# bensonlzl/spaced-kmer-sketching

Measured on AMD Instinct MI355X. Metric: k-mers hashed/s + genome-pairs ANI/s at 1/2/4/8 MI355X; % HBM roofline, higher is better.
Workload: dtype u64; 1 GPU; config3: 1x3 Gb multi-contig genome per GPU, spaced seed w=31/k=21 (mask seed 0), FracMinHash 1/1000; builds_in_flight=3, genome_bytes=3000000024, windows_per_genome=2999036400, sketch_size=2998764, parallelism=genome-sharded x1

## Files before the change

spaced-kmer-sketching_amd/csrc/scan.hip:

```cpp
#include <hip/hip_runtime.h>

#include <cstdlib>

#include <cstdint>
#include <type_traits>

#include "code_objects.hpp"
#include "scan.hpp"
#include "sks_hash.hpp"

namespace sks {

namespace {

constexpr int kBlock = 256;
constexpr int kWPT = 16;
constexpr int kTile = kBlock * kWPT;
constexpr int kHaloWords = 4;
constexpr int kWords = kBlock + kHaloWords;
constexpr int kLoadVecs = (kWords * 16 + 16) / 16;
constexpr int kQCap = 2048;
#ifndef SKS_SCAN_QCAP
#define SKS_SCAN_QCAP 512
#endif
template <int MODE>
constexpr int qcap() { return MODE == kModeList ? kQCap : SKS_SCAN_QCAP; }
constexpr unsigned char kSep = '\n';

struct Geom {
  uint64_t win0;
  uint64_t seg_end;
  uint32_t seg;
};

__device__ __forceinline__ Geom tile_geom(const ScanParams& p, uint64_t tile, uint32_t& seg) {
  while (seg + 1 < p.n_seg && tile >= p.tile_prefix[seg + 1]) ++seg;
  Geom g;
  g.seg = seg;
  g.win0 = p.seg_begin[seg] + (tile - p.tile_prefix[seg]) * (uint64_t)kTile;
  g.seg_end = p.seg_end[seg];
  return g;
}

__device__ __forceinline__ uint4 load_vec(const uint8_t* __restrict__ seq, int64_t base, int k,
                                          int64_t seg_end) {
  int64_t a = base + 16 * (int64_t)k;
  if (a + 16 <= seg_end) return *reinterpret_cast<const uint4*>(seq + a);
  uint32_t wv[4];
#pragma unroll
  for (int q = 0; q < 4; ++q) {
    uint32_t v = 0;
#pragma unroll
    for (int b = 0; b < 4; ++b) {
      int64_t pos = a + 4 * q + b;
      uint32_t ch = pos < seg_end ? seq[pos] : kSep;
      v |= ch << (8 * b);
    }
    wv[q] = v;
  }
  return make_uint4(wv[0], wv[1], wv[2], wv[3]);
}

__device__ __forceinline__ uint32_t align_shift(const uint8_t* seq, uint64_t win0) {
  return (uint32_t)(((uintptr_t)seq + win0) & 15u);
}

__device__ __forceinline__ void encode4(uint32_t x, uint32_t& le8, uint32_t& inv4) {
  uint32_t low = x | 0x20202020u;
  uint32_t code = ((low >> 1) ^ (low >> 2)) & 0x03030303u;
  uint32_t expect = __builtin_amdgcn_perm(0u, 0x74676361u, code);
  uint32_t eq = expect ^ low;
  uint32_t t = (eq & 0x7F7F7F7Fu) + 0x7F7F7F7Fu;
  t = ~(t | eq | 0x7F7F7F7Fu);
  uint32_t bad = (~t) & 0x80808080u;
  inv4 = (bad * 0x00204081u) >> 28;
  uint32_t y = code | (code >> 6);
  le8 = (y | (y >> 12)) & 0xFFu;
}

__device__ __forceinline__ uint32_t funnel(uint32_t hi, uint32_t lo, uint32_t s) {
  return __builtin_amdgcn_alignbit(hi, lo, s);
}

template <bool ALIGNED>
__device__ __forceinline__ void pack16(const uint32_t (&x)[5], uint32_t sb, uint32_t& le,
                                       uint32_t& inv) {
  uint32_t w[4], g[4], sad = 0;
#pragma unroll
  for (int k = 0; k < 4; ++k) {
    w[k] = ALIGNED ? x[k] : funnel(x[k + 1], x[k], sb);
    const uint32_t low = w[k] | 0x20202020u;
    const uint32_t code = ((low >> 1) ^ (low >> 2)) & 0x03030303u;
    const uint32_t expect = __builtin_amdgcn_perm(0u, 0x74676361u, code);
    sad = __builtin_amdgcn_sad_u8(low, expect, sad);
    g[k] = code * 0x01041040u;
  }
  const uint32_t g01 = __builtin_amdgcn_perm(g[1], g[0], 0x0c0c0703u);
  const uint32_t g23 = __builtin_amdgcn_perm(g[3], g[2], 0x0c0c0703u);
  le = __builtin_amdgcn_perm(g23, g01, 0x05040100u);
  inv = 0;
  if (sad) {
#pragma unroll
    for (int k = 0; k < 4; ++k) {
      uint32_t le8, inv4;
      encode4(w[k], le8, inv4);
      inv |= inv4 << (4 * k);
    }
  }
}

__device__ __forceinline__ uint32_t rev_pairs(uint32_t x) {
  uint32_t r = __builtin_bitreverse32(x);
  return ((r >> 1) & 0x55555555u) | ((r & 0x55555555u) << 1);
}


__device__ __forceinline__ unsigned long long wave_aggregated_inc(unsigned long long* counter) {
  const uint64_t act = __ballot(true);
  const uint32_t rank = __builtin_amdgcn_mbcnt_hi((uint32_t)(act >> 32),
                                                  __builtin_amdgcn_mbcnt_lo((uint32_t)act, 0u));
  unsigned long long base = 0;
  if (rank == 0) base = atomicAdd(counter, (unsigned long long)__popcll(act));
  const uint32_t lo = __builtin_amdgcn_readfirstlane((uint32_t)base);
  const uint32_t hi = __builtin_amdgcn_readfirstlane((uint32_t)(base >> 32));
  return (((unsigned long long)hi << 32) | lo) + rank;
}

template <int MODE>
struct Queue {
  uint64_t key[qcap<MODE>()];
  uint64_t val[MODE == kModeBottom ? qcap<MODE>() : 1];
  uint32_t n;
  unsigned long long base;
  unsigned long long wins;
};

template <int MODE>
__device__ __forceinline__ void emit(const ScanParams& p, Queue<MODE>& q, uint32_t seg,
                                     uint64_t key, uint64_t val) {
  uint32_t slot = atomicAdd(&q.n, 1u);
  if (slot < (uint32_t)qcap<MODE>()) {
    q.key[slot] = key;
    if constexpr (MODE == kModeBottom) q.val[slot] = val;
  } else {
    unsigned long long g = wave_aggregated_inc(&p.seg_count[seg]);
    if (g < p.seg_out_cap[seg]) {
      uint64_t o = p.seg_out_off[seg] + g;
      p.out_key[o] = key;
      if constexpr (MODE == kModeBottom) p.out_val[o] = val;
    }
  }
}

template <int MODE>
__device__ __forceinline__ void flush(const ScanParams& p, Queue<MODE>& q, uint32_t seg) {
  __syncthreads();
  if (threadIdx.x == 0 && q.wins) atomicAdd(&p.seg_windows[seg], q.wins);
  constexpr uint32_t cap = qcap<MODE>();
  uint32_t n = q.n < cap ? q.n : cap;
  if (n) {
    if (threadIdx.x == 0) q.base = atomicAdd(&p.seg_count[seg], (unsigned long long)n);
    __syncthreads();
    uint64_t base = q.base;
    uint64_t cap = p.seg_out_cap[seg];
    uint64_t off = p.seg_out_off[seg];
    for (uint32_t i = threadIdx.x; i < n; i += kBlock) {
      if (base + i < cap) {
        p.out_key[off + base + i] = q.key[i];
        if constexpr (MODE == kModeBottom) p.out_val[off + base + i] = q.val[i];
      }
    }
  }
  __syncthreads();
  if (threadIdx.x == 0) {
    q.n = 0;
    q.wins = 0;
  }
  __syncthreads();
}

__device__ __forceinline__ void add_windows(unsigned long long& wins, uint32_t cnt) {
  uint32_t v = cnt;
#pragma unroll
  for (int o = 32; o > 0; o >>= 1) v += __shfl_xor(v, o, 64);
  if ((threadIdx.x & 63) == 0 && v) atomicAdd(&wins, (unsigned long long)v);
}

template <int FLAVOUR>
__device__ __forceinline__ uint64_t fmh_narrow(const ScanParams& p, uint64_t c) {
  uint64_t h;
  if constexpr (FLAVOUR == 0) {
    h = hash_mix(c + kGolden32);
    h = hash_mix(h + kGolden32);
    h = hash_mix(h + (128 + kGolden32));
  } else {
    h = hash_bitset128<1>(c, 0);
  }
  return h ^ p.kconst;
}

__device__ __forceinline__ uint64_t mix3_head(uint64_t c) {
  uint64_t h = hash_mix(c + kGolden32);
  h = hash_mix(h + kGolden32);
  uint64_t x = h + (128 + kGolden32);
  x ^= x >> 32;
  x = mul_const<kMixMul>(x);
  return x ^ (x >> 32);
}

template <int MODE>
__device__ __forceinline__ bool keep_fmh(const ScanParams& p, uint64_t f, uint64_t thresh) {
  if constexpr (MODE != kModeBottom) return div_test(f, p.low_mask, p.high_mask, p.dinv, p.dlim);
  else return f <= thresh;
}

constexpr int kBeOff = 2;

template <int MODE, int PRE>
constexpr int min_waves() {
#ifdef SKS_SCAN_MIN_WAVES
  return SKS_SCAN_MIN_WAVES;
#else
  return PRE ? 7 : MODE == kModeList ? 4 : 5;
#endif
}

constexpr uint32_t kCandCap = 128;

constexpr int kFminMaxW = 31;
__device__ __forceinline__ uint64_t min_below_2_62(uint64_t a, uint64_t b) {
  uint64_t r;
  asm("v_min_f64 %0, %1, %2" : "=v"(r) : "v"(a), "v"(b));
  return r;
}

template <int MODE, int FLAVOUR, int PRE = 0, int FMIN = 0>
__global__ __launch_bounds__(kBlock, (min_waves<MODE, PRE>())) void scan_kernel(ScanParams p) {
  __shared__ uint32_t s_raw[kLoadVecs * 4];
  __shared__ uint32_t s_be[kWords + 2 + kBeOff];
  __shared__ uint32_t s_lc[kWords + 2];
  __shared__ uint32_t s_inv[kWords + 2];
  __shared__ Queue<MODE> q;
  __shared__ ulonglong2 s_cand[PRE ? (kBlock / 64) * kCandCap : 1];
  __shared__ uint32_t s_ctop[PRE ? kBlock / 64 : 1];

  __shared__ unsigned long long s_next;

  const int tid = threadIdx.x;
  const bool dyn = p.tile_queue != nullptr;
  uint64_t t_begin, t_end;
  if (dyn) {
    t_begin = (uint64_t)blockIdx.x * p.chunk;
    t_end = min(t_begin + p.chunk, p.n_tiles);
  } else {
    t_begin = (uint64_t)blockIdx.x * p.n_tiles / gridDim.x;
    t_end = (uint64_t)(blockIdx.x + 1) * p.n_tiles / gridDim.x;
  }
  if (tid == 0) {
    q.n = 0;
    q.wins = 0;
  }
  if (t_begin >= t_end) return;
  unsigned long long grab = 0;

  const int w = p.w;
  const uint32_t dshift = 2 * (32 - w);
  const uint64_t wmask_bits = (w >= 64) ? ~0ull : ((1ull << w) - 1);
  if (tid < kBeOff) s_be[tid] = 0;
  const uint32_t r = tid & 15;
  const uint32_t wbase = (uint32_t)(tid >> 4) * kWPT;
  const uint32_t of = 2 * r + 64 - dshift;
  const uint32_t qf = (of - 1) >> 5;
  const uint32_t sF = 32 * qf + 32 - of;
  const uint32_t sR = 2 * r;
  const uint32_t* const fb = s_be + (kBeOff - 2) + wbase + qf;
  const uint32_t* const rb = s_lc + wbase;

  uint32_t seg_lo = 0, seg_hi = p.n_seg;
  while (seg_lo + 1 < seg_hi) {
    uint32_t mid = (seg_lo + seg_hi) >> 1;
    if (p.tile_prefix[mid] <= t_begin) seg_lo = mid; else seg_hi = mid;
  }
  uint32_t cur_seg = seg_lo, pf_seg = seg_lo;

  Geom pg = tile_geom(p, t_begin, pf_seg);
  int64_t pf_base = (int64_t)pg.win0 - align_shift(p.seq, pg.win0);
  uint4 v0 = load_vec(p.seq, pf_base, tid, (int64_t)pg.seg_end);
  uint4 v1 = make_uint4(0, 0, 0, 0);
  if (tid < kLoadVecs - kBlock) v1 = load_vec(p.seq, pf_base, kBlock + tid, (int64_t)pg.seg_end);

  uint32_t win_count = 0;
  uint32_t count_seg = cur_seg;

  for (uint64_t tile = t_begin; tile < t_end;) {
    Geom g = tile_geom(p, tile, cur_seg);
    if (g.seg != count_seg) {
      add_windows(q.wins, win_count);
      win_count = 0;
      flush<MODE>(p, q, count_seg);
      count_seg = g.seg;
    }
    const uint32_t shift = align_shift(p.seq, g.win0);
    const uint64_t thresh = (MODE == kModeBottom) ? p.seg_thresh[g.seg] : 0;
    const bool last_of_chunk = tile + 1 == t_end;
    if (dyn && tid == 0) {
      if (tile == t_begin)
        grab = (unsigned long long)gridDim.x * p.chunk + atomicAdd(p.tile_queue, (unsigned long long)p.chunk);
      if (last_of_chunk) s_next = grab;
    }

    auto store_word = [&](int i, uint32_t le, uint32_t inv) {
      s_be[kBeOff + i] = rev_pairs(le);
      s_lc[i] = ~le;
      s_inv[i] = inv;
    };
    if (shift == 0) {
      uint32_t le, inv;
      const uint32_t x0[5] = {v0.x, v0.y, v0.z, v0.w, 0u};
      pack16<true>(x0, 0, le, inv);
      store_word(tid, le, inv);
      if (tid < kHaloWords) {
        const uint32_t x1[5] = {v1.x, v1.y, v1.z, v1.w, 0u};
        pack16<true>(x1, 0, le, inv);
        store_word(kBlock + tid, le, inv);
      }
    } else {
      reinterpret_cast<uint4*>(s_raw)[tid] = v0;
      if (tid < kLoadVecs - kBlock) reinterpret_cast<uint4*>(s_raw)[kBlock + tid] = v1;
      __syncthreads();
      const uint32_t sb = (shift & 3) * 8;
      for (int i = tid; i < kWords; i += kBlock) {
        const uint32_t wi = (16 * i + shift) >> 2;
        uint32_t x[5];
#pragma unroll
        for (int k = 0; k < 5; ++k) x[k] = s_raw[wi + k];
        uint32_t le, inv;
        pack16<false>(x, sb, le, inv);
        store_word(i, le, inv);
      }
    }
    __syncthreads();
    uint64_t next_tile = !last_of_chunk ? tile + 1 : p.n_tiles;
    if (last_of_chunk && dyn) {
      const unsigned long long sn = s_next;
      next_tile = ((uint64_t)__builtin_amdgcn_readfirstlane((uint32_t)(sn >> 32)) << 32) |
                  __builtin_amdgcn_readfirstlane((uint32_t)sn);
    }

    if (next_tile < (dyn ? p.n_tiles : t_end)) {
      Geom ng = tile_geom(p, next_tile, pf_seg);
      pf_base = (int64_t)ng.win0 - align_shift(p.seq, ng.win0);
      v0 = load_vec(p.seq, pf_base, tid, (int64_t)ng.seg_end);
      if (tid < kLoadVecs - kBlock) v1 = load_vec(p.seq, pf_base, kBlock + tid, (int64_t)ng.seg_end);
    }

    const int lane = tid & 63;
    bool dirty = s_inv[tid] != 0;
    if (lane < 2) dirty = dirty || s_inv[(tid | 63) + 1 + lane] != 0;
    const bool wave_clean = !__any(dirty);
    auto canon_of = [&](uint32_t fh, uint32_t fl, uint32_t rh, uint32_t rl) -> uint64_t {
      const uint64_t F = (((uint64_t)fh) << 32) | fl;
      const uint64_t R = (((uint64_t)rh) << 32) | rl;
      const uint64_t fm = F & p.mask_lo, rm = R & p.mask_lo;
      if constexpr (FMIN) return min_below_2_62(fm, rm);
      else return fm < rm ? fm : rm;
    };
    auto canon_at = [&](uint32_t m) -> uint64_t {
      const uint32_t f0 = fb[m], f1 = fb[m + 1], f2 = fb[m + 2];
      const uint32_t r0 = rb[m], r1 = rb[m + 1], r2 = rb[m + 2];
      return canon_of(funnel(f0, f1, sF), funnel(f1, f2, sF), funnel(r2, r1, sR), funnel(r1, r0, sR));
    };
    auto for_windows_checked = [&](auto body) {
      const uint32_t* const ib = s_inv + wbase;
      uint32_t fw = fb[1], rw = rb[1];
      uint32_t fp = funnel(fb[0], fw, sF), rp = funnel(rw, rb[0], sR);
      uint32_t i0 = ib[0], i1 = ib[1];
      uint32_t fnext = 0, rnext = 0, inext = 0;
      if constexpr (!PRE) {
        fnext = fb[2];
        rnext = rb[2];
        inext = ib[2];
      }
#pragma unroll 1
      for (int m = 0; m < kWPT; ++m) {
        uint32_t fw2, rw2, i2;
        if constexpr (PRE) {
          fw2 = fb[m + 2];
          rw2 = rb[m + 2];
          i2 = ib[m + 2];
        } else {
          fw2 = fnext;
          rw2 = rnext;
          i2 = inext;
          fnext = fb[m + 3];
          rnext = rb[m + 3];
          inext = ib[m + 3];
        }
        const uint32_t fn = funnel(fw, fw2, sF), rn = funnel(rw2, rw, sR);
        const uint64_t iv = (uint64_t)i0 | ((uint64_t)i1 << 16) | ((uint64_t)i2 << 32);
        body(m, canon_of(fp, fn, rn, rp), ((iv >> r) & wmask_bits) == 0);
        fw = fw2; rw = rw2; fp = fn; rp = rn; i0 = i1; i1 = i2;
      }
    };
    auto for_windows = [&](auto body) {
      uint32_t fw = fb[1], rw = rb[1];
      uint32_t fp = funnel(fb[0], fw, sF), rp = funnel(rw, rb[0], sR);
      uint32_t fnext = fb[2], rnext = rb[2];
#pragma unroll
      for (int m = 0; m < kWPT; ++m) {
        const uint32_t fw2 = fnext, rw2 = rnext;
        if (m + 1 < kWPT) {
          fnext = fb[m + 3];
          rnext = rb[m + 3];
        }
        asm volatile("" ::: "memory");
        const uint32_t fn = funnel(fw, fw2, sF), rn = funnel(rw2, rw, sR);
        body(m, canon_of(fp, fn, rn, rp));
        fw = fw2; rw = rw2; fp = fn; rp = rn;
      }
    };
    if constexpr (PRE) {
      const uint32_t wv = __builtin_amdgcn_readfirstlane(tid >> 6);
      ulonglong2* cb = s_cand + wv * kCandCap;
      uint32_t* const ctop = s_ctop + wv;
      typedef unsigned long long u64x2 __attribute__((ext_vector_type(2)));
      typedef __attribute__((address_space(3))) u64x2 lds_u64x2;
      const uint32_t cb_lds = (uint32_t)(uintptr_t)(__attribute__((address_space(3))) void*)cb;
      auto set_cursor = [&](uint32_t n) {
        if (lane == 0) *ctop = cb_lds + 16 * n;
        __builtin_amdgcn_fence(__ATOMIC_RELEASE, "wavefront");
        __builtin_amdgcn_wave_barrier();
        __builtin_amdgcn_fence(__ATOMIC_ACQUIRE, "wavefront");
      };
      const uint32_t pmask = p.low_mask & 0xFu;
      const uint32_t kbits = (uint32_t)p.kconst & pmask;
      const uint32_t rest_lo = p.low_mask & ~0xFu, rest_hi = p.high_mask;
      uint32_t cnt = 0;
      set_cursor(0);
      auto finish = [&](uint32_t n) {
        __builtin_amdgcn_wave_barrier();
        if ((uint32_t)lane < n) {
          const ulonglong2 e = cb[lane];
          uint64_t y = mul_const<kMixMul>(e.x);
          y ^= y >> 28;
          const uint64_t f = y ^ p.kconst;
          bool keep = mul_uniform(f, p.dinv) <= p.dlim;
          if (rest_lo | rest_hi)
            keep = keep && ((((uint32_t)f & rest_lo) | ((uint32_t)(f >> 32) & rest_hi)) == 0);
          if (keep) emit<MODE>(p, q, g.seg, e.y, 0);
        }
        __builtin_amdgcn_wave_barrier();
      };
      auto window_pre = [&](uint64_t c, bool valid) {
          const uint64_t z = mix3_head(c);
          const uint32_t ylo = (uint32_t)z * (uint32_t)kMixMul;
          const bool pass = (((ylo ^ (ylo >> 28)) & pmask) == kbits) && valid;
          const uint64_t bal = __ballot(pass);
          if (pass) {
            const uint32_t slot = atomicAdd(ctop, 16u);
            u64x2 zc;
            zc.x = z;
            zc.y = c;
            *(lds_u64x2*)(uintptr_t)slot = zc;
          }
          cnt += (uint32_t)__popcll(bal);
          if (cnt >= 64) {
            finish(64);
            const uint32_t rest = cnt - 64;
            ulonglong2 t = make_ulonglong2(0, 0);
            if ((uint32_t)lane < rest) t = cb[64 + lane];
            __builtin_amdgcn_wave_barrier();
            if ((uint32_t)lane < rest) cb[lane] = t;
            cnt = rest;
            set_cursor(rest);
          }
      };
      if (wave_clean) {
        for_windows([&](int, uint64_t c) { window_pre(c, true); });
        win_count += kWPT;
      } else {
        for_windows_checked([&](int, uint64_t c, bool valid) {
          win_count += valid ? 1u : 0u;
          window_pre(c, valid);
        });
      }
      if (cnt) finish(cnt);
    } else {
    uint32_t keepmask = 0;
    const uint32_t thr_top = (uint32_t)(thresh >> 36);
    const uint32_t k_top = (uint32_t)(p.kconst >> 32);
    auto keep_window = [&](uint64_t c) -> bool {
      if constexpr (MODE == kModeBottom && FLAVOUR == 0) {
        const uint64_t y = mul_const<kMixMul>(mix3_head(c));
        return (((uint32_t)(y >> 32) ^ k_top) >> 4) <= thr_top;
      } else {
        return keep_fmh<MODE>(p, fmh_narrow<FLAVOUR>(p, c), thresh);
      }
    };
    if (wave_clean) {
      for_windows([&](int m, uint64_t c) { keepmask |= (keep_window(c) ? 1u : 0u) << m; });
      win_count += kWPT;
    } else {
      for_windows_checked([&](int m, uint64_t c, bool valid) {
        win_count += valid ? 1u : 0u;
        keepmask |= (keep_window(c) && valid ? 1u : 0u) << m;
      });
    }
    while (keepmask) {
      const uint32_t j = __builtin_ctz(keepmask);
      keepmask &= keepmask - 1;
      if constexpr (MODE == kModeList) {
        emit<MODE>(p, q, g.seg, g.win0 + (uint64_t)(16 * (wbase + j) + r), 0);
      } else {
        const uint64_t c = canon_at(j);
        if constexpr (MODE == kModeFrac) emit<MODE>(p, q, g.seg, c, 0);
        else emit<MODE>(p, q, g.seg, c, c);
      }
    }
    }

    __syncthreads();
    if (q.n >= (uint32_t)qcap<MODE>() / 2) {
      add_windows(q.wins, win_count);
      win_count = 0;
      flush<MODE>(p, q, g.seg);
    }
    if (!last_of_chunk) {
      ++tile;
    } else if (dyn) {
      t_begin = tile = next_tile;
      t_end = min(next_tile + p.chunk, p.n_tiles);
    } else {
      break;
    }
  }
  add_windows(q.wins, win_count);
  flush<MODE>(p, q, count_seg);
}

template <int MODE, int FLAVOUR>
__global__ __launch_bounds__(kBlock) void scan_kernel_wide(ScanParams p) {
  __shared__ uint32_t s_raw[kLoadVecs * 4];
  __shared__ uint32_t s_be[kWords + 2];
  __shared__ uint32_t s_lc[kWords + 2];
  __shared__ uint32_t s_inv[kWords + 2];
  __shared__ uint64_t q_a[kQCap / 2], q_b[kQCap / 2], q_c[kQCap / 2];
  __shared__ uint32_t q_n;
  __shared__ unsigned long long q_base, q_wins;

  const int tid = threadIdx.x;
  const uint64_t t_begin = (uint64_t)blockIdx.x * p.n_tiles / gridDim.x;
  const uint64_t t_end = (uint64_t)(blockIdx.x + 1) * p.n_tiles / gridDim.x;
  if (tid == 0) {
    q_n = 0;
    q_wins = 0;
  }
  if (t_begin >= t_end) return;
  constexpr uint32_t cap = kQCap / 2;

  const int w = p.w;
  const uint32_t fshift = 128 - 2 * w;
  const uint64_t wmask_bits = (w >= 64) ? ~0ull : ((1ull << w) - 1);

  uint32_t seg_lo = 0, seg_hi = p.n_seg;
  while (seg_lo + 1 < seg_hi) {
    uint32_t mid = (seg_lo + seg_hi) >> 1;
    if (p.tile_prefix[mid] <= t_begin) seg_lo = mid; else seg_hi = mid;
  }
  uint32_t cur_seg = seg_lo, pf_seg = seg_lo;
  Geom pg = tile_geom(p, t_begin, pf_seg);
  int64_t pf_base = (int64_t)pg.win0 - align_shift(p.seq, pg.win0);
  uint4 v0 = load_vec(p.seq, pf_base, tid, (int64_t)pg.seg_end);
  uint4 v1 = make_uint4(0, 0, 0, 0);
  if (tid < kLoadVecs - kBlock) v1 = load_vec(p.seq, pf_base, kBlock + tid, (int64_t)pg.seg_end);
  uint32_t win_count = 0;
  uint32_t count_seg = cur_seg;

  auto wflush = [&](uint32_t seg) {
    __syncthreads();
    if (tid == 0 && q_wins) atomicAdd(&p.seg_windows[seg], q_wins);
    uint32_t n = q_n < cap ? q_n : cap;
    if (n) {
      if (tid == 0) q_base = atomicAdd(&p.seg_count[seg], (unsigned long long)n);
      __syncthreads();
      uint64_t base = q_base, c = p.seg_out_cap[seg], off = p.seg_out_off[seg];
      for (uint32_t i = tid; i < n; i += kBlock)
        if (base + i < c) {
          p.out_key[off + base + i] = q_a[i];
          if (MODE != kModeList) p.out_val[off + base + i] = q_b[i];
          if (MODE == kModeBottom) p.out_hi[off + base + i] = q_c[i];
        }
    }
    __syncthreads();
    if (tid == 0) {
      q_n = 0;
      q_wins = 0;
    }
    __syncthreads();
  };

  for (uint64_t tile = t_begin; tile < t_end; ++tile) {
    Geom g = tile_geom(p, tile, cur_seg);
    if (g.seg != count_seg) {
      add_windows(q_wins, win_count);
      win_count = 0;
      wflush(count_seg);
      count_seg = g.seg;
    }
    const uint32_t shift = align_shift(p.seq, g.win0);
    const uint64_t thresh = (MODE == kModeBottom) ? p.seg_thresh[g.seg] : 0;
    reinterpret_cast<uint4*>(s_raw)[tid] = v0;
    if (tid < kLoadVecs - kBlock) reinterpret_cast<uint4*>(s_raw)[kBlock + tid] = v1;
    __syncthreads();
    for (int i = tid; i < kWords; i += kBlock) {
      const uint32_t b0 = 16 * i + shift;
      const uint32_t wi = b0 >> 2, sb = (b0 & 3) * 8;
      uint32_t x[5];
#pragma unroll
      for (int k = 0; k < 5; ++k) x[k] = s_raw[wi + k];
      uint32_t le, inv;
      pack16<false>(x, sb, le, inv);
      s_be[i] = rev_pairs(le);
      s_lc[i] = ~le;
      s_inv[i] = inv;
    }
    __syncthreads();
    if (tile + 1 < t_end) {
      Geom ng = tile_geom(p, tile + 1, pf_seg);
      pf_base = (int64_t)ng.win0 - align_shift(p.seq, ng.win0);
      v0 = load_vec(p.seq, pf_base, tid, (int64_t)ng.seg_end);
      if (tid < kLoadVecs - kBlock) v1 = load_vec(p.seq, pf_base, kBlock + tid, (int64_t)ng.seg_end);
    }
    uint32_t be[5], lc[5];
#pragma unroll
    for (int k = 0; k < 5; ++k) { be[k] = s_be[tid + k]; lc[k] = s_lc[tid + k]; }
    const uint64_t inv_lo = (uint64_t)s_inv[tid] | ((uint64_t)s_inv[tid + 1] << 16) |
                            ((uint64_t)s_inv[tid + 2] << 32) | ((uint64_t)s_inv[tid + 3] << 48);
    const uint64_t inv_hi = (uint64_t)s_inv[tid + 4];
#pragma unroll
    for (int j = 0; j < kWPT; ++j) {
      uint32_t f3 = j ? funnel(be[0], be[1], 32 - 2 * j) : be[0];
      uint32_t f2 = j ? funnel(be[1], be[2], 32 - 2 * j) : be[1];
      uint32_t f1 = j ? funnel(be[2], be[3], 32 - 2 * j) : be[2];
      uint32_t f0 = j ? funnel(be[3], be[4], 32 - 2 * j) : be[3];
      uint64_t Fh = ((uint64_t)f3 << 32) | f2, Fl = ((uint64_t)f1 << 32) | f0;
      if (fshift) { Fl = (Fl >> fshift) | (Fh << (64 - fshift)); Fh >>= fshift; }
      uint32_t r0 = j ? funnel(lc[1], lc[0], 2 * j) : lc[0];
      uint32_t r1 = j ? funnel(lc[2], lc[1], 2 * j) : lc[1];
      uint32_t r2 = j ? funnel(lc[3], lc[2], 2 * j) : lc[2];
      uint32_t r3 = j ? funnel(lc[4], lc[3], 2 * j) : lc[3];
      uint64_t Rl = ((uint64_t)r1 << 32) | r0, Rh = ((uint64_t)r3 << 32) | r2;
      uint64_t fml = Fl & p.mask_lo, fmh = Fh & p.mask_hi;
      uint64_t rml = Rl & p.mask_lo, rmh = Rh & p.mask_hi;
      bool f_lt = (fmh < rmh) || (fmh == rmh && fml < rml);
      uint64_t cl = f_lt ? fml : rml, ch = f_lt ? fmh : rmh;
      uint64_t iv = (inv_lo >> j) | (j ? (inv_hi << (64 - j)) : 0);
      bool valid = (iv & wmask_bits) == 0;
      win_count += valid ? 1u : 0u;
      uint64_t h;
      if constexpr (FLAVOUR == 0) {
        h = hash_mix(cl + kGolden32);
        h = hash_mix(h + kGolden32 + ch);
        h = hash_mix(h + (128 + kGolden32));
      } else {
        h = hash_bitset128<1>(cl, ch);
      }
      uint64_t f = h ^ p.kconst;
      bool keep = (MODE != kModeBottom) ? div_test(f, p.low_mask, p.high_mask, p.dinv, p.dlim)
                                        : (f <= thresh);
      if (valid && keep) {
        uint32_t slot = atomicAdd(&q_n, 1u);
        uint64_t a = (MODE == kModeList) ? g.win0 + (uint64_t)(kWPT * tid) + j
                                         : (MODE == kModeFrac) ? cl : f;
        uint64_t b = (MODE == kModeFrac) ? ch : cl;
        if (slot < cap) {
          q_a[slot] = a; q_b[slot] = b; q_c[slot] = ch;
        } else {
          unsigned long long gi = wave_aggregated_inc(&p.seg_count[g.seg]);
          if (gi < p.seg_out_cap[g.seg]) {
            uint64_t o = p.seg_out_off[g.seg] + gi;
            p.out_key[o] = a;
            if (MODE != kModeList) p.out_val[o] = b;
            if (MODE == kModeBottom) p.out_hi[o] = ch;
          }
        }
      }
    }
    __syncthreads();
    if (q_n >= cap / 2) {
      add_windows(q_wins, win_count);
      win_count = 0;
      wflush(g.seg);
    }
  }
  add_windows(q_wins, win_count);
  wflush(count_seg);
}

template <int MODE, int FLAVOUR, int PRE, class Run>
hipError_t run_narrow(const ScanParams& p, Run run) {
  return p.w <= kFminMaxW ? run(scan_kernel<MODE, FLAVOUR, PRE, 1>) : run(scan_kernel<MODE, FLAVOUR, PRE, 0>);
}

constexpr int kGridOversubscribe = 16;
constexpr int kDynOversubscribe = 2;

template <class K>
int occupancy_grid(K kernel, int device) {
  int per_cu = 0;
  (void)hipOccupancyMaxActiveBlocksPerMultiprocessor(&per_cu, kernel, kBlock, 0);
  int cus = 0;
  (void)hipDeviceGetAttribute(&cus, hipDeviceAttributeMultiprocessorCount, device);
  if (per_cu < 1) per_cu = 1;
  if (cus < 1) cus = 1;
  return per_cu * cus;
}

}

uint64_t scan_tiles_for(uint64_t seg_bytes) { return (seg_bytes + kTile - 1) / kTile; }

hipError_t launch_scan(const ScanParams& p, int mode, int flavour, bool wide, int device,
                       hipStream_t stream, int grid_override) {
  if (p.n_tiles == 0) return hipSuccess;
  auto pick = [&](auto kernel) -> hipError_t {
    ScanParams q = p;
    q.tile_queue = nullptr;
    int grid = grid_override > 0 ? grid_override : kGridOversubscribe * occupancy_grid(kernel, device);
    if ((uint64_t)grid > p.n_tiles) grid = (int)p.n_tiles;
    hipLaunchKernelGGL(kernel, dim3(grid), dim3(kBlock), 0, stream, q);
    return hipGetLastError();
  };
  auto pick_dyn = [&](auto kernel) -> hipError_t {
    ScanParams q = p;
    int grid = grid_override > 0 ? grid_override : kDynOversubscribe * occupancy_grid(kernel, device);
    const uint64_t per = p.n_tiles / ((uint64_t)grid * 16);
    static const uint64_t min_chunk = getenv("SKS_SCAN_MIN_CHUNK") ? std::max(1, atoi(getenv("SKS_SCAN_MIN_CHUNK"))) : 3;
    q.chunk = (uint32_t)std::min<uint64_t>(16, std::max<uint64_t>(min_chunk, per));
    const uint64_t need = (p.n_tiles + q.chunk - 1) / q.chunk;
    if ((uint64_t)grid > need) grid = (int)need;
    hipLaunchKernelGGL(kernel, dim3(grid), dim3(kBlock), 0, stream, q);
    return hipGetLastError();
  };
  if (!wide && p.tile_queue) {
    if (mode == kModeFrac) {
      static const bool no_pre = getenv("SKS_NO_PREFILTER") != nullptr;
      if (flavour == 0 && (p.low_mask & 0xFu) && !no_pre) return run_narrow<kModeFrac, 0, 1>(p, pick_dyn);
      return flavour == 0 ? run_narrow<kModeFrac, 0, 0>(p, pick_dyn) : run_narrow<kModeFrac, 1, 0>(p, pick_dyn);
    }
    if (mode == kModeBottom)
      return flavour == 0 ? run_narrow<kModeBottom, 0, 0>(p, pick_dyn) : run_narrow<kModeBottom, 1, 0>(p, pick_dyn);
  }
  if (!wide) {
    if (mode == kModeFrac) {
      static const bool no_pre = getenv("SKS_NO_PREFILTER") != nullptr;
      if (flavour == 0 && (p.low_mask & 0xFu) && !no_pre) return run_narrow<kModeFrac, 0, 1>(p, pick);
      return flavour == 0 ? run_narrow<kModeFrac, 0, 0>(p, pick) : run_narrow<kModeFrac, 1, 0>(p, pick);
    }
    if (mode == kModeList) return flavour == 0 ? pick(scan_kernel<kModeList, 0>) : pick(scan_kernel<kModeList, 1>);
    return flavour == 0 ? run_narrow<kModeBottom, 0, 0>(p, pick) : run_narrow<kModeBottom, 1, 0>(p, pick);
  }
  if (mode == kModeFrac) return flavour == 0 ? pick(scan_kernel_wide<kModeFrac, 0>) : pick(scan_kernel_wide<kModeFrac, 1>);
  if (mode == kModeList) return flavour == 0 ? pick(scan_kernel_wide<kModeList, 0>) : pick(scan_kernel_wide<kModeList, 1>);
  return flavour == 0 ? pick(scan_kernel_wide<kModeBottom, 0>) : pick(scan_kernel_wide<kModeBottom, 1>);
}

SKS_CODE_OBJECT_HOOK(scan)

}
```

Before: 772.4 billion k-mers/s.

## Keep tile geometry in scalar registers and streamline prefetch and candidate handling

Replaces per-tile segment lookup with a scalar-resident SegCursor that carries segment begin, end and threshold, and precomputes the next tile's geometry during prefetch. The common interior case uses an unguarded global load with an SGPR base. The candidate buffer is addressed through a per-lane LDS pointer, and the candidate copy no longer goes through a temporary with an extra wave barrier. The FMH filter uses bitop3 and funnel shifts, and min waves are raised to 6 for the bottom-k FMIN variant. Together these cut VALU and scalar overhead and load latency, at the cost of relying on inline asm constraints and the register pressure that comes with higher occupancy.

```diff
diff --git a/spaced-kmer-sketching_amd/csrc/scan.hip b/spaced-kmer-sketching_amd/csrc/scan.hip
--- a/spaced-kmer-sketching_amd/csrc/scan.hip
+++ b/spaced-kmer-sketching_amd/csrc/scan.hip
@@ -42,10 +42,80 @@
   return g;
 }
 
-__device__ __forceinline__ uint4 load_vec(const uint8_t* __restrict__ seq, int64_t base, int k,
-                                          int64_t seg_end) {
+__device__ __forceinline__ uint64_t uniform64(uint64_t v) {
+  const uint32_t lo = (uint32_t)__builtin_amdgcn_readfirstlane((uint32_t)v);
+  const uint32_t hi = (uint32_t)__builtin_amdgcn_readfirstlane((uint32_t)(v >> 32));
+  return ((uint64_t)hi << 32) | lo;
+}
+
+__device__ __forceinline__ uint64_t own_sgprs(uint64_t v) {
+  asm("" : "+s"(v));
+  return v;
+}
+
+__device__ __forceinline__ bool uniform_less(uint64_t a, uint64_t b) {
+  uint32_t diff, borrow;
+  asm("s_sub_u32 %0, %2, %4\n\ts_subb_u32 %0, %3, %5\n\ts_cselect_b32 %1, 1, 0"
+      : "=&s"(diff), "=s"(borrow)
+      : "s"((uint32_t)a), "s"((uint32_t)(a >> 32)), "s"((uint32_t)b), "s"((uint32_t)(b >> 32))
+      : "scc");
+  return borrow != 0;
+}
+
+template <int MODE>
+struct SegCursor {
+  uint32_t seg;
+  uint64_t next_prefix;
+  uint64_t win_off;
+  int64_t end;
+  uint64_t thresh;
+
+  __device__ __forceinline__ void load(const ScanParams& p, uint64_t prefix) {
+    win_off = uniform64(p.seg_begin[seg]) - prefix * (uint64_t)kTile;
+    end = (int64_t)uniform64(p.seg_end[seg]);
+    if constexpr (MODE == kModeBottom) thresh = uniform64(p.seg_thresh[seg]);
+  }
+  __device__ __forceinline__ void start(const ScanParams& p, uint32_t s) {
+    seg = __builtin_amdgcn_readfirstlane(s);
+    next_prefix = uniform64(p.tile_prefix[seg + 1]);
+    load(p, uniform64(p.tile_prefix[seg]));
+  }
+  __device__ __forceinline__ void seek(const ScanParams& p, uint64_t tile) {
+    if (seg + 1 < p.n_seg && !uniform_less(tile, next_prefix)) {
+      uint64_t prefix;
+      do {
+        ++seg;
+        prefix = next_prefix;
+        next_prefix = uniform64(p.tile_prefix[seg + 1]);
+      } while (seg + 1 < p.n_seg && !uniform_less(tile, next_prefix));
+      load(p, prefix);
+    }
+  }
+};
+
+struct TileGeom {
+  uint64_t win0;
+  uint64_t thresh;
+  uint32_t seg;
+  uint32_t shift;
+};
+
+typedef const __attribute__((address_space(1))) uint8_t* GlobalBytes;
+__device__ __forceinline__ GlobalBytes global_bytes(uint64_t address) {
+  return reinterpret_cast<GlobalBytes>((uintptr_t)address);
+}
+
+__device__ __forceinline__ uint4 load16(const uint8_t* at) { return *reinterpret_cast<const uint4*>(at); }
+__device__ __forceinline__ uint4 load16(GlobalBytes at) {
+  typedef uint32_t u32x4 __attribute__((ext_vector_type(4)));
+  const u32x4 v = *reinterpret_cast<const __attribute__((address_space(1))) u32x4*>(at);
+  return make_uint4(v.x, v.y, v.z, v.w);
+}
+
+template <class Bytes>
+__device__ __forceinline__ uint4 load_vec(Bytes seq, int64_t base, int k, int64_t seg_end) {
   int64_t a = base + 16 * (int64_t)k;
-  if (a + 16 <= seg_end) return *reinterpret_cast<const uint4*>(seq + a);
+  if (a + 16 <= seg_end) return load16(seq + a);
   uint32_t wv[4];
 #pragma unroll
   for (int q = 0; q < 4; ++q) {
@@ -61,8 +131,9 @@
   return make_uint4(wv[0], wv[1], wv[2], wv[3]);
 }
 
-__device__ __forceinline__ uint32_t align_shift(const uint8_t* seq, uint64_t win0) {
-  return (uint32_t)(((uintptr_t)seq + win0) & 15u);
+template <class Bytes>
+__device__ __forceinline__ uint32_t align_shift(Bytes seq, uint64_t win0) {
+  return (uint32_t)(((uint64_t)(uintptr_t)seq + win0) & 15u);
 }
 
 __device__ __forceinline__ void encode4(uint32_t x, uint32_t& le8, uint32_t& inv4) {
@@ -216,12 +287,12 @@
 
 constexpr int kBeOff = 2;
 
-template <int MODE, int PRE>
+template <int MODE, int PRE, int FMIN>
 constexpr int min_waves() {
 #ifdef SKS_SCAN_MIN_WAVES
   return SKS_SCAN_MIN_WAVES;
 #else
-  return PRE ? 7 : MODE == kModeList ? 4 : 5;
+  return PRE ? 7 : MODE == kModeList ? 4 : (MODE == kModeBottom && FMIN) ? 6 : 5;
 #endif
 }
 
@@ -235,7 +306,7 @@
 }
 
 template <int MODE, int FLAVOUR, int PRE = 0, int FMIN = 0>
-__global__ __launch_bounds__(kBlock, (min_waves<MODE, PRE>())) void scan_kernel(ScanParams p) {
+__global__ __launch_bounds__(kBlock, (min_waves<MODE, PRE, FMIN>())) void scan_kernel(ScanParams p) {
   __shared__ uint32_t s_raw[kLoadVecs * 4];
   __shared__ uint32_t s_be[kWords + 2 + kBeOff];
   __shared__ uint32_t s_lc[kWords + 2];
@@ -281,29 +352,58 @@
     uint32_t mid = (seg_lo + seg_hi) >> 1;
     if (p.tile_prefix[mid] <= t_begin) seg_lo = mid; else seg_hi = mid;
   }
-  uint32_t cur_seg = seg_lo, pf_seg = seg_lo;
-
-  Geom pg = tile_geom(p, t_begin, pf_seg);
-  int64_t pf_base = (int64_t)pg.win0 - align_shift(p.seq, pg.win0);
-  uint4 v0 = load_vec(p.seq, pf_base, tid, (int64_t)pg.seg_end);
-  uint4 v1 = make_uint4(0, 0, 0, 0);
-  if (tid < kLoadVecs - kBlock) v1 = load_vec(p.seq, pf_base, kBlock + tid, (int64_t)pg.seg_end);
+  SegCursor<MODE> sc;
+  sc.start(p, seg_lo);
+  const GlobalBytes seq = global_bytes(own_sgprs((uint64_t)(uintptr_t)p.seq));
+  TileGeom pg;
+  uint4 v0, v1 = make_uint4(0, 0, 0, 0);
+  auto prefetch = [&](uint64_t t) {
+    sc.seek(p, t);
+    pg.seg = sc.seg;
+    pg.thresh = (MODE == kModeBottom) ? sc.thresh : 0;
+    pg.win0 = sc.win_off + t * (uint64_t)kTile;
+    pg.shift = align_shift(seq, pg.win0);
+    const int64_t base = (int64_t)pg.win0 - pg.shift;
+    const bool interior = !uniform_less((uint64_t)sc.end, (uint64_t)(base + 16 * kLoadVecs));
+    const uint64_t bp = (uint64_t)(uintptr_t)seq + (uint64_t)base;
+    uint32_t lane_off = 16 * tid;
+    asm volatile("" : "+v"(lane_off));
+    if (interior) v0 = load16(global_bytes(own_sgprs(bp)) + lane_off);
+    else v0 = load_vec(seq, base, tid, sc.end);
+    if (lane_off < 16 * (kLoadVecs - kBlock)) {
+      if (interior) {
+        asm volatile("" : "+v"(lane_off));
+        v1 = load16(global_bytes(own_sgprs(bp + 16 * kBlock)) + lane_off);
+      } else {
+        v1 = load_vec(seq, base, kBlock + tid, sc.end);
+      }
+    }
+  };
+  prefetch(t_begin);
 
   uint32_t win_count = 0;
-  uint32_t count_seg = cur_seg;
+  uint32_t count_seg = pg.seg;
+
+  uint32_t cb_lane = 0;
+  if constexpr (PRE) {
+    cb_lane = (uint32_t)(uintptr_t)(__attribute__((address_space(3))) void*)(s_cand + (tid >> 6) * kCandCap + (tid & 63));
+    asm volatile("" : "+v"(cb_lane));
+  }
 
   for (uint64_t tile = t_begin; tile < t_end;) {
-    Geom g = tile_geom(p, tile, cur_seg);
+    const TileGeom g = pg;
+    int ltid = tid;
+    asm volatile("" : "+v"(ltid));
     if (g.seg != count_seg) {
       add_windows(q.wins, win_count);
       win_count = 0;
       flush<MODE>(p, q, count_seg);
       count_seg = g.seg;
     }
-    const uint32_t shift = align_shift(p.seq, g.win0);
-    const uint64_t thresh = (MODE == kModeBottom) ? p.seg_thresh[g.seg] : 0;
+    const uint32_t shift = g.shift;
+    const uint64_t thresh = g.thresh;
     const bool last_of_chunk = tile + 1 == t_end;
-    if (dyn && tid == 0) {
+    if (dyn && ltid == 0) {
       if (tile == t_begin)
         grab = (unsigned long long)gridDim.x * p.chunk + atomicAdd(p.tile_queue, (unsigned long long)p.chunk);
       if (last_of_chunk) s_next = grab;
@@ -319,7 +419,7 @@
       const uint32_t x0[5] = {v0.x, v0.y, v0.z, v0.w, 0u};
       pack16<true>(x0, 0, le, inv);
       store_word(tid, le, inv);
-      if (tid < kHaloWords) {
+      if (ltid < kHaloWords) {
         const uint32_t x1[5] = {v1.x, v1.y, v1.z, v1.w, 0u};
         pack16<true>(x1, 0, le, inv);
         store_word(kBlock + tid, le, inv);
@@ -340,19 +440,14 @@
       }
     }
     __syncthreads();
-    uint64_t next_tile = !last_of_chunk ? tile + 1 : p.n_tiles;
+    uint64_t next_tile = tile + 1;
+    bool more = !last_of_chunk;
     if (last_of_chunk && dyn) {
-      const unsigned long long sn = s_next;
-      next_tile = ((uint64_t)__builtin_amdgcn_readfirstlane((uint32_t)(sn >> 32)) << 32) |
-                  __builtin_amdgcn_readfirstlane((uint32_t)sn);
-    }
-
-    if (next_tile < (dyn ? p.n_tiles : t_end)) {
-      Geom ng = tile_geom(p, next_tile, pf_seg);
-      pf_base = (int64_t)ng.win0 - align_shift(p.seq, ng.win0);
-      v0 = load_vec(p.seq, pf_base, tid, (int64_t)ng.seg_end);
-      if (tid < kLoadVecs - kBlock) v1 = load_vec(p.seq, pf_base, kBlock + tid, (int64_t)ng.seg_end);
-    }
+      next_tile = uniform64(s_next);
+      more = uniform_less(next_tile, p.n_tiles);
+    }
+
+    if (more) prefetch(next_tile);
 
     const int lane = tid & 63;
     bool dirty = s_inv[tid] != 0;
@@ -432,6 +527,7 @@
         __builtin_amdgcn_wave_barrier();
         __builtin_amdgcn_fence(__ATOMIC_ACQUIRE, "wavefront");
       };
+      auto cand_at = [&](uint32_t i) { return (lds_u64x2*)(uintptr_t)(cb_lane + 16 * i); };
       const uint32_t pmask = p.low_mask & 0xFu;
       const uint32_t kbits = (uint32_t)p.kconst & pmask;
       const uint32_t rest_lo = p.low_mask & ~0xFu, rest_hi = p.high_mask;
@@ -440,14 +536,18 @@
       auto finish = [&](uint32_t n) {
         __builtin_amdgcn_wave_barrier();
         if ((uint32_t)lane < n) {
-          const ulonglong2 e = cb[lane];
-          uint64_t y = mul_const<kMixMul>(e.x);
-          y ^= y >> 28;
-          const uint64_t f = y ^ p.kconst;
-          bool keep = mul_uniform(f, p.dinv) <= p.dlim;
-          if (rest_lo | rest_hi)
-            keep = keep && ((((uint32_t)f & rest_lo) | ((uint32_t)(f >> 32) & rest_hi)) == 0);
-          if (keep) emit<MODE>(p, q, g.seg, e.y, 0);
+          const u64x2 e = *cand_at(0);
+          const uint64_t y = mul_const<kMixMul>(e.x);
+          const uint32_t ylo = (uint32_t)y, yhi = (uint32_t)(y >> 32);
+          const uint32_t flo = __builtin_amdgcn_bitop3_b32(ylo, funnel(yhi, ylo, 28), (uint32_t)p.kconst, 0x96);
+          const uint32_t fhi = __builtin_amdgcn_bitop3_b32(yhi, yhi >> 28, (uint32_t)(p.kconst >> 32), 0x96);
+          const uint64_t f = ((uint64_t)fhi << 32) | flo;
+          if (mul_uniform(f, p.dinv) <= p.dlim) {
+            bool keep = true;
+            if (rest_lo | rest_hi)
+              keep = ((flo & rest_lo) | (fhi & rest_hi)) == 0;
+            if (keep) emit<MODE>(p, q, g.seg, e.y, 0);
+          }
         }
         __builtin_amdgcn_wave_barrier();
       };
@@ -467,10 +567,7 @@
           if (cnt >= 64) {
             finish(64);
             const uint32_t rest = cnt - 64;
-            ulonglong2 t = make_ulonglong2(0, 0);
-            if ((uint32_t)lane < rest) t = cb[64 + lane];
-            __builtin_amdgcn_wave_barrier();
-            if ((uint32_t)lane < rest) cb[lane] = t;
+            if ((uint32_t)lane < rest) *cand_at(0) = *cand_at(64);
             cnt = rest;
             set_cursor(rest);
           }
```

Result: faster. 792.9 billion k-mers/s, median of 6 (+2.7%).
